# indrajeetadityaroy9/vit-inductive-bias-distillation

Measured on AMD Instinct MI355X. Metric: distillation images/sec (BASD loss fwd+bwd+grad all-reduce), DeiT-S<-ResNet-50 @ bs256/GPU, higher is better.
Workload: dtype f32; 1 GPU; cfg2 DeiT-S<-ResNet-50 224x224; per_gpu_batch=256, global_batch=256, input_dtype=float32, layout=strided (CLS-sliced / channel-major views), backward=True, grad_allreduce_bytes=88202672, grad_allreduce=none at world size 1 (bucket packed, nothing to exchange), rank_readback=auto, readback_deferred_steps=1756, selector=basd_selector_chain mode 0, parallelism=dp1

## Files before the change

### include/basd_hip.h

```cpp
#ifndef BASD_HIP_H
#define BASD_HIP_H

#include <stdint.h>

#ifdef __cplusplus
extern "C" {
#endif

#ifndef __HIP_PLATFORM_AMD__
typedef struct ihipStream_t* hipStream_t;
#endif

#define BASD_OK 0
#define BASD_EINVAL (-1)
#define BASD_EUNSUPPORTED (-2)
#define BASD_DTYPE_F32 0
#define BASD_DTYPE_BF16 1
#define BASD_DTYPE_U8 2


int basd_gemm_nt(const void* a, int a_dtype, long a_sb, long a_sn, long a_sd, int a_rows_per_batch,
                 long a_batch_stride, const float* b, long ldb, long b_batch_stride, int M, int N, int K, int batch,
                 float* c, long ldc, long c_batch_stride, float scale, const float* bias, float beta,
                 float* colsum_part, float* col_mean, hipStream_t stream);
// ... 153 lines not shown
                              const float* omega_t, float* mu, float* tc, hipStream_t stream);
long basd_teacher_center_stream_scratch_floats(int G, int B, int n, int D);
int basd_teacher_center_stream(const void* const* tok_ptrs, int dtype, const float* mix, int L, int G, long sb, long sn,
                               long sd, int B, int n, int D, const int* g0, const int* g1, const float* glam,
                               const float* omega_t, float* mu, float* tc, float* scratch, hipStream_t stream);

int basd_gram_f64(const float* p, long p_batch_stride, int n, int D, int batch, double* g, long g_batch_stride,
                  hipStream_t stream);

int basd_gram_f64_split(const float* p, long p_batch_stride, int n, int D, int batch, int splits, double* slabs,
                        double* g, hipStream_t stream);

int basd_chol_f64(const double* g, long g_batch_stride, int n, int batch, double* l, long l_batch_stride,
                  hipStream_t stream);

int basd_stack_product(const double* la, const double* lb, long l_batch_stride, int n, int batch, int lb_period,
                       float* w, long w_batch_stride, hipStream_t stream);

int basd_procrustes_finalize(const float* w, long w_batch_stride, const float* sigma, int n, int n_s, int batch,
                             int t_period ,
                             const double* gb, long g_batch_stride, const float* omega, const int* tap0,
                             const int* tap1, const float* lam, const float* tr_s_part, int tr_slabs, float* tr_s,
                             float* tr_t, float* nuc, float* loss, float* k_prime, hipStream_t stream);

int basd_student_project_multi(const void* const* x_ptrs, int dtype, long sb, long sn, int E, int B, int n_s, int n_t,
                               int D, int ptrs_16B_aligned, const float* omega, long omega_e_stride, const int* tap0,
                               const int* tap1, const float* lam, const int* range0, const int* range1, float* mu,
                               float* tr_s, float* a_prime, hipStream_t stream);
int basd_student_grad_multi(const void* const* x_ptrs, int dtype, long sb, long sn, int E, int B, int n_s, int n_t,
                            int D, const float* omega, long omega_e_stride, const float* mu, const float* h,
// ... 32 lines not shown
int basd_procrustes_forward_fused(const BasdProcrustesArgs* args, hipStream_t stream);
int basd_procrustes_tuning(int transposed_cores);

int basd_stack_product_t(const double* la, const double* lb, long l_batch_stride, int n, int batch, int lb_period,
                         float* w, long w_batch_stride, hipStream_t stream);
int basd_kprime_from_transposed(const float* w, long w_batch_stride, const float* sigma, int n, int batch,
                                const double* lb, long l_batch_stride, int lb_period, float* z, long z_batch_stride,
                                float* k_prime, hipStream_t stream);
int basd_procrustes_finish_transposed(const float* w, long w_batch_stride, const float* sigma, int n, int n_s,
                                      int batch, int t_period ,
                                      const double* gb, long g_batch_stride, const float* omega, const int* tap0,
                                      const int* tap1, const float* lam, const float* tr_s_part, int tr_slabs,
                                      float* tr_s, float* tr_t, float* nuc, float* loss, const double* lb,
                                      long l_batch_stride, int lb_period, float* k_prime, hipStream_t stream);
int basd_procrustes_finish_tuning(int fused);
int basd_ustack_stash(const float* wc, long wc_batch_stride, int n, int batch, float* w_stack, long w_stack_stride,
                      hipStream_t stream);
int basd_ustack_from_transposed(const float* x, long x_batch_stride, const float* sigma, int n, int batch,
                                float* w_stack, long w_stack_stride, float* scratch, long scratch_batch_stride,
                                float* sigma_u, int max_sweeps, int* jflags, hipStream_t stream);

int basd_scale_unless_one(float* x, long count, const float* num, const float* den, hipStream_t stream);

int basd_cross_entropy(const void* logits, int dtype, long ld, int B, int C, const long* labels, const float* probs,
                       long pld, float label_smoothing, long ignore_index, float* row_loss, float* dlogits,
                       hipStream_t stream);


int basd_event_create(void** out);
int basd_event_destroy(void* event);
// ... 156 lines not shown
```

### vit-inductive-bias-distillation_amd/basd_amd/_lib.py

```python
from __future__ import annotations

import ctypes as C
import os
import threading

_HERE = os.path.dirname(os.path.abspath(__file__))
LIB_PATH = os.path.join(_HERE, "libbasd_hip.so")

vp, i32, i64, f32, f64 = C.c_void_p, C.c_int, C.c_long, C.c_float, C.c_double

SIGNATURES = {
    "basd_gemm_nt": [vp, i32, i64, i64, i64, i32, i64, vp, i64, i64, i32, i32, i32, i32, vp, i64, i64, f32, vp, f32,
                     vp, vp, vp],
    "basd_gemm_tn_splits": [i32],
    "basd_gemm_tn": [vp, vp, i32, i64, i64, i64, i64, i64, i64, i64, i64, i32, i32, i32, i32, i32, vp, vp, i32, vp,
                     vp, i64, i64, f32, vp],
    "basd_colmean_parts": [i32],
    "basd_colmean": [vp, i32, i64, i64, i64, i32, i64, i32, i32, i32, i32, vp, vp, vp],
    "basd_colmean_multi": [vp, i32, i64, i64, i64, i32, i32, i32, i32, i32, vp, vp, i32, vp],
    "basd_syrk_splits": [i32, i32, i32],
    "basd_syrk_multi": [vp, i32, i64, i64, i64, i32, i32, i32, i32, vp, vp, i32, vp, vp, i64, i32, vp, i32, i32, vp],
    "basd_jacobi_workspace_ints": [i32, i32],
    "basd_jacobi_max_rows": [],
    "basd_jacobi_twopass_workspace_bytes": [i32, i32, i32],
# ... 42 lines not shown
                                 vp, vp],
    "basd_student_project_multi": [vp, i32, i64, i64, i32, i32, i32, i32, i32, i32, vp, i64, vp, vp, vp, vp, vp, vp,
                                   vp, vp, vp],
    "basd_student_grad_multi": [vp, i32, i64, i64, i32, i32, i32, i32, i32, vp, i64, vp, vp, vp, vp, vp, vp, f32, vp,
                                vp, vp, vp],
    "basd_student_grad_fused": [vp, i32, i64, i64, i32, i32, i32, i32, i32, i32, vp, i64, vp, vp, vp, vp, vp, vp, vp,
                                f32, vp, vp],
    "basd_procrustes_forward_fused": [vp, vp],
    "basd_procrustes_tuning": [i32],
    "basd_jacobi_plain4_fits": [i32],
    "basd_stack_product_t": [vp, vp, i64, i32, i32, i32, vp, i64, vp],
    "basd_kprime_from_transposed": [vp, i64, vp, i32, i32, vp, i64, i32, vp, i64, vp, vp],
    "basd_procrustes_finish_transposed": [vp, i64, vp, i32, i32, i32, i32, vp, i64, vp, vp, vp, vp, vp, i32, vp, vp, vp,
                                          vp, vp, i64, i32, vp, vp],
    "basd_procrustes_finish_tuning": [i32],
    "basd_ustack_stash": [vp, i64, i32, i32, vp, i64, vp],
    "basd_ustack_from_transposed": [vp, i64, vp, i32, i32, vp, i64, vp, i64, vp, i32, vp, vp],
    "basd_resample_tokens": [vp, i32, i64, i64, i64, i32, i32, i32, i32, vp, vp, vp, vp, vp],
    "basd_resample_tokens_adjoint": [vp, i32, i32, i32, i32, vp, vp, vp, vp, vp, vp, vp],
    "basd_teacher_factor": [vp, i64, vp, i32, i32, i32, vp, vp, i64, vp, vp, vp, vp, vp, vp, vp, vp, vp],
    "basd_teacher_factor_tiled": [vp, i64, vp, i32, i32, i32, vp, vp, i64, vp, vp, vp, vp, vp, vp, vp, vp, vp, vp],
    "basd_mix_grad_tokens": [vp, vp, i32, i32, i64, i64, i64, i32, i32, i32, i32, vp, vp, vp, vp, vp],
    "basd_mix_grad_tokens_scratch_floats": [i32, i32, i32, i32],
    "basd_mix_grad_tokens_onepass": [vp, vp, i32, i32, i64, i64, i64, i32, i32, i32, i32, vp, vp, vp, vp, vp, vp],
    "basd_token_weight_bwd": [vp, vp, i32, i32, i32, i32, vp, vp, vp, vp, vp, vp, i32, i32, i64, i64, i64, i64, i32,
                              i32, i32, vp, vp, vp],
    "basd_build_angle_stack": [vp, i32, vp, i32, vp, vp],
    "basd_grassmann_distance_bwd": [vp, vp, i32, vp, vp, i32, vp, vp, i32, vp, vp],
    "basd_eigvec_k2": [vp, vp, i32, i32, i32, vp, vp],
    "basd_selector_chain": [vp],
# ... 114 lines not shown
```

### vit-inductive-bias-distillation_amd/csrc/fused.hip

```cpp
#include "basd_common.h"
#include "../../include/basd_hip.h"

namespace basd {

__global__ void __launch_bounds__(256) uwso_combine_kernel(const float* __restrict__ ce, const float* __restrict__ loss_b,
                                                           int E, int B, float* __restrict__ out) {
    constexpr int CH = 32;
    __shared__ double red[CH][4];
    const int tid = threadIdx.x;
    double geo_sum = 0.;
    for (int e0 = 0; e0 < E; e0 += CH) {
        const int ne = E - e0 < CH ? E - e0 : CH;
        for (int e = 0; e < ne; ++e) {
            double acc = 0.;
            for (int b = tid; b < B; b += 256) acc += (double)loss_b[(long)(e0 + e) * B + b];
            for (int m = 32; m > 0; m >>= 1) acc += __shfl_xor(acc, m, 64);
            if ((tid & 63) == 0) red[e][tid >> 6] = acc;
        }
        __syncthreads();
        if (tid == 0)
            for (int e = 0; e < ne; ++e) {
                const float layer = (float)(((red[e][0] + red[e][1]) + (red[e][2] + red[e][3])) / (double)B);
                out[4 + E + e0 + e] = layer;
                geo_sum += (double)layer;
// ... 1 lines not shown
        __syncthreads();
    }
    if (tid == 0) {
        const float c = ce[0], geo = (float)(geo_sum / (double)E);
        const float eps = 1.1920929e-7f;
        const float i0 = 1.f / fmaxf(c, eps), i1 = 1.f / fmaxf(geo, eps);
        const float w0 = i0 / (i0 + i1), w1 = i1 / (i0 + i1);
        out[0] = w0;
        out[1] = w1;
        out[2] = w0 * c + w1 * geo;
        out[3] = geo;
        for (int e = 0; e < E; ++e) out[4 + e] = w1 / (float)E;
    }
}

__global__ void __launch_bounds__(256) scale_unless_one_kernel(float* __restrict__ x, long count4, long count,
                                                               const float* __restrict__ num,
                                                               const float* __restrict__ den) {
    const float f = den ? num[0] / den[0] : num[0];
    if (f == 1.f) return;
    const long i = (long)blockIdx.x * 256 + threadIdx.x;
    if (i < count4) {
        float4 v = ((float4*)x)[i];
        v.x *= f; v.y *= f; v.z *= f; v.w *= f;
        ((float4*)x)[i] = v;
    }
    if (blockIdx.x == 0 && threadIdx.x < (int)(count - 4 * count4)) x[4 * count4 + threadIdx.x] *= f;
}

}

extern "C" {

int basd_scale_unless_one(float* x, long count, const float* num, const float* den, hipStream_t stream) {
    BASD_CHECK_ARG(x && num && count > 0 && ((uintptr_t)x & 15) == 0);
    const long count4 = count / 4;
    basd::scale_unless_one_kernel<<<(unsigned)((count4 + 255) / 256 + (count4 == 0)), 256, 0, stream>>>(x, count4, count, num, den);
    BASD_RETURN_LAST();
}

static int procrustes_tail(const BasdProcrustesArgs* a, const float* grad_layers, int E, int B, int n_s, int n, int d_s,
                           int EB, long nn, long om_stride, hipStream_t st) {
    int rc;
#define BASD_TRY(call)            \
    do {                          \
        rc = (call);              \
        if (rc != BASD_OK) return rc; \
    } while (0)
    if (a->uw_ce) {
        BASD_CHECK_ARG(a->uw_out != nullptr);
        basd::uwso_combine_kernel<<<1, 256, 0, st>>>(a->uw_ce, a->loss_b, E, B, a->uw_out);
        grad_layers = a->uw_out + 4;
// ... 65 lines not shown
    rc = basd_student_project_multi(a->student_ptrs, (int)a->s_dtype, a->s_sb, a->s_sn, E, B, n_s, n, d_s,
                                    (int)a->s_aligned, a->omega, om_stride, a->tap0, a->tap1, a->lam, a->range0,
                                    a->range1, a->mu_s, a->tr_part, a->a_prime, st);
    if (rc == BASD_EUNSUPPORTED) {
        slabs = (d_s + 63) / 64;
        for (int e = 0; e < E; ++e)
            BASD_TRY(basd_student_project(a->student_host_ptrs[e], (int)a->s_dtype, a->s_sb, a->s_sn, B, n_s, n, d_s,
                                          a->omega + e * om_stride, a->tap0, a->tap1, a->lam, a->range0, a->range1,
                                          a->mu_s + (long)e * B * d_s, a->tr_part + (long)e * B * slabs,
                                          a->a_prime + (long)e * B * n * d_s, st));
    } else if (rc != BASD_OK) {
        return rc;
    }
    const long nn = (long)n * n;
    const int EB = E * B, GB = G * B;
    BASD_TRY(basd_gram_f64(a->a_prime, (long)n * d_s, n, d_s, EB, a->g_all, nn, st));
    if (a->g_slabs && a->g_splits > 1)
        BASD_TRY(basd_gram_f64_split(a->tc, (long)n * d_t, n, d_t, GB, (int)a->g_splits, a->g_slabs,
                                     a->g_all + (long)EB * nn, st));
    else
        BASD_TRY(basd_gram_f64(a->tc, (long)n * d_t, n, d_t, GB, a->g_all + (long)EB * nn, nn, st));
    BASD_TRY(basd_chol_f64(a->g_all, nn, n, EB + GB, a->l_all, nn, st));
    if ((a->raw == nullptr || a->w_stack != nullptr) && EB <= 65535 && basd_jacobi_plain4_fits(n) &&
        (g_transposed_cores == 2 || (g_transposed_cores == 1 && EB >= 128))) {
        BASD_TRY(basd_stack_product_t(a->l_all, a->l_all + (long)EB * nn, nn, n, EB, GB, a->W, 2 * nn, st));
        if (a->raw != nullptr) BASD_TRY(basd_ustack_stash(a->W, 2 * nn, n, EB, a->w_stack, 2 * nn, st));
        BASD_TRY(basd_jacobi_onesided(a->W, 2 * nn, n, n, n, EB, nullptr, a->sigma, n, (int)a->max_sweeps, 0.f,
                                      a->jflags, a->sweeps, st));
        rc = BASD_EUNSUPPORTED;
        if (a->k_prime && g_finish_fused)
            rc = basd_procrustes_finish_transposed(a->W, 2 * nn, a->sigma, n, n_s, EB, GB, a->g_all + (long)EB * nn, nn,
                                                   a->omega, a->tap0, a->tap1, a->lam, a->tr_part, slabs, a->tr_s,
                                                   a->tr_t, a->nuc, a->loss_b, a->l_all + (long)EB * nn, nn, GB,
                                                   a->k_prime, st);
        if (rc == BASD_EUNSUPPORTED) {
            BASD_TRY(basd_procrustes_finalize(a->W, 2 * nn, a->sigma, n, n_s, EB, GB, a->g_all + (long)EB * nn, nn,
                                              a->omega, a->tap0, a->tap1, a->lam, a->tr_part, slabs, a->tr_s, a->tr_t,
// ... 48 lines not shown
```

### vit-inductive-bias-distillation_amd/csrc/jacobi.hip

```cpp
#include "basd_common.h"

namespace basd {

constexpr float kNull2 = 2.2737368e-13f;

struct Rot {
    float c, s, t;
    float h;
    bool apply;
    bool strong;
};

__device__ __forceinline__ Rot make_rotation(float alpha, float beta, float gamma, float tol) {
    Rot r{1.f, 0.f, 0.f, 0.f, false, false};
    const float cosv = gamma * __builtin_amdgcn_rsqf(alpha) * __builtin_amdgcn_rsqf(beta);
    if (!(fabsf(cosv) > tol)) return r;
    r.strong = cosv * cosv > tol;
    const float zeta = (beta - alpha) * __builtin_amdgcn_rcpf(2.f * gamma);
    const float az = fabsf(zeta);
    float t = az > 1e8f ? 0.5f * __builtin_amdgcn_rcpf(az)
                        : __builtin_amdgcn_rcpf(az + __builtin_amdgcn_sqrtf(fmaf(zeta, zeta, 1.f)));
    t = copysignf(t, zeta);
    r.t = t;
    r.c = __builtin_amdgcn_rsqf(fmaf(t, t, 1.f));
// ... 767 lines not shown
            (void)hipFuncSetAttribute((const void*)jacobi_lds_kernel<20, 20, 8>,
                                      hipFuncAttributeMaxDynamicSharedMemorySize, BASD_JACOBI_LDS_LIMIT);
            jacobi_lds_kernel<20, 20, 8><<<batch, threads, lds8p, stream>>>(W, batch_stride, rows_dot, rows_tot, n, n_arr,
                                                                            max_sweeps, tol, colnorm, colnorm_stride,
                                                                            sweeps_out);
            BASD_RETURN_LAST();
        }
    }

    if (g_jacobi_ordering == 1 && !stacked && !n_arr && n_even >= 8 && rows_tot == rows_dot &&
        (lanes == 0 || lanes == 4) && (g_jacobi_lanes == 4 || (batch >= 128 && n_even >= 40) || n_even >= 96)) {
        static const int o_epl[] = {8, 16, 24, 36, 50};
        int e4 = 0;
        for (int e : o_epl)
            if (4 * e >= rows_tot) { e4 = e; break; }
        const int G = n_even / 2;
        const size_t lds_oe = (size_t)(G + 1) * (plain4_ld(e4) + 2) * sizeof(float);
        const int threads = ((G * 4 + 63) / 64) * 64;
        if (e4 && threads <= 512 && lds_oe <= BASD_JACOBI_LDS_LIMIT) {
#define LAUNCH_OE(E)                                                                                                  \
    do {                                                                                                              \
        if (lds_oe > 48 * 1024)                                                                                       \
            (void)hipFuncSetAttribute((const void*)jacobi_oe_kernel<E>, hipFuncAttributeMaxDynamicSharedMemorySize,   \
                                      BASD_JACOBI_LDS_LIMIT);                                                         \
        jacobi_oe_kernel<E><<<batch, threads, lds_oe, stream>>>(W, batch_stride, rows_tot, n, max_sweeps, tol, colnorm, \
                                                                colnorm_stride, sweeps_out);                          \
    } while (0)
            switch (e4) {
                case 8: LAUNCH_OE(8); break;
                case 16: LAUNCH_OE(16); break;
                case 24: LAUNCH_OE(24); break;
                case 36: LAUNCH_OE(36); break;
                default: LAUNCH_OE(50); break;
            }
#undef LAUNCH_OE
            BASD_RETURN_LAST();
        }
    }

    if (!stacked && !n_arr && n_even >= 8 && (lanes == 4 || (lanes == 0 && batch >= 128 && n_even >= 40))) {
        static const int p_epl[] = {8, 16, 24, 36, 50};
        int e4 = 0;
        for (int e : p_epl)
            if (4 * e >= rows_tot) { e4 = e; break; }
// ... 233 lines not shown
```

### vit-inductive-bias-distillation_amd/csrc/procrustes.hip

```cpp
#include "basd_common.h"
#include "../../include/basd_hip.h"

namespace basd {

typedef double f64x4 __attribute__((ext_vector_type(4)));

template <typename T>
__global__ void __launch_bounds__(256) token_weights_kernel(const void* const* __restrict__ attn_ptrs,
                                                            const float* __restrict__ mix, int L, long sb, long sh,
                                                            long sq, long sk, int H, int A, int has_cls, int n_a,
                                                            int n_t, int n_s, const int* __restrict__ atap0,
                                                            const int* __restrict__ atap1,
                                                            const float* __restrict__ alam,
                                                            const int* __restrict__ tap0,
                                                            const int* __restrict__ tap1,
                                                            const float* __restrict__ lam, float* __restrict__ omega,
                                                            float* __restrict__ omega_t, float* __restrict__ raw_out) {
    extern __shared__ float sm[];
    float* raw = sm;
    float* w = sm + n_a;
    __shared__ float red[32];
    const int b = blockIdx.x, tid = threadIdx.x;
    for (int j = tid; j < n_a; j += blockDim.x) {
        float acc = 0.f;
// ... 6 lines not shown
            }
            acc /= (float)H;
        } else {
            for (int h = 0; h < H; ++h)
                for (int q = 0; q < A; ++q) {
                    float m = 0.f;
                    for (int l = 0; l < L; ++l)
                        m += mix[l] * ldg_f32((const BASD_GLOBAL_AS T*)attn_ptrs[l] + (b * sb + h * sh + q * sq + (long)j * sk));
                    acc += m;
                }
            acc /= (float)(H * A);
        }
        raw[j] = acc;
        if (raw_out) raw_out[(long)b * n_a + j] = acc;
    }
    __syncthreads();
    float part = 0.f;
    for (int n = tid; n < n_s; n += blockDim.x) {
        float v;
        if (atap0) {
            const float l1 = alam[n];
            v = (1.f - l1) * raw[atap0[n]] + l1 * raw[atap1[n]];
        } else {
            v = raw[n];
        }
        w[n] = v;
        part += v;
    }
    const float total = block_sum(part, red);
    for (int n = tid; n < n_s; n += blockDim.x) {
        const float v = w[n] / total;
        w[n] = v;
        omega[(long)b * n_s + n] = v;
    }
    __syncthreads();
    for (int j = tid; j < n_t; j += blockDim.x) {
        float acc = 0.f;
        if (tap0) {
            for (int n = 0; n < n_s; ++n) {
                const float l1 = lam[n];
                if (tap0[n] == j) acc += (1.f - l1) * w[n];
                if (tap1[n] == j) acc += l1 * w[n];
            }
        } else {
            acc = w[j];
        }
        omega_t[(long)b * n_t + j] = acc;
    }
}

template <typename T>
__global__ void __launch_bounds__(256) student_project_kernel(const T* __restrict__ X, long sb, long sn, int n_s,
                                                              int n_t, int D, const float* __restrict__ omega,
                                                              const int* __restrict__ tap0,
                                                              const int* __restrict__ tap1,
                                                              const float* __restrict__ lam,
                                                              const int* __restrict__ range0,
                                                              const int* __restrict__ range1,
                                                              float* __restrict__ mu_out, float* __restrict__ tr_part,
                                                              float* __restrict__ Ap) {
    extern __shared__ float sm[];
    float* w = sm;
    __shared__ float red[4][64];
// ... 376 lines not shown
                                                                   int D, float* __restrict__ mu_out,
                                                                   float* __restrict__ Tc) {
    const int d = blockIdx.x * 256 + threadIdx.x, chunk = blockIdx.y;
    const long gb = blockIdx.z, GB = gridDim.z;
    if (d >= D) return;
    float mu = 0.f;
    for (int c = 0; c < chunks; ++c) mu += chunk_sum[((long)c * GB + gb) * D + d];
    if (chunk == 0) mu_out[gb * D + d] = mu;
    const int j_lo = chunk * TCS_ROWS, j_hi = j_lo + TCS_ROWS < n ? j_lo + TCS_ROWS : n;
    float* out = Tc + gb * n * D + d;
    for (int j = j_lo; j < j_hi; ++j) out[(long)j * D] -= mu;
}

constexpr int G64_BK = 32, G64_LD = 36, G64_TPW = 8;

__global__ void __launch_bounds__(1024) gram_f64_kernel(const float* __restrict__ P, long p_batch_stride, int n, int D,
                                                        double* __restrict__ G, long g_batch_stride,
                                                        long g_split_stride) {
    extern __shared__ __attribute__((aligned(16))) float tile[];
    const int b = blockIdx.x, tid = threadIdx.x, lane = tid & 63, wave = tid >> 6, nw = blockDim.x >> 6;
    G += (long)blockIdx.y * g_split_stride;
    const int nt = (n + 15) / 16, ntiles = nt * (nt + 1) / 2;
    const float* Pb = P + (long)b * p_batch_stride;
    f64x4 acc[G64_TPW];
#pragma unroll
    for (int t = 0; t < G64_TPW; ++t) acc[t] = f64x4{0., 0., 0., 0.};
    int ti[G64_TPW], tj[G64_TPW];
#pragma unroll
    for (int t = 0; t < G64_TPW; ++t) {
        const int lin = wave + (t + (int)blockIdx.z * G64_TPW) * nw;
        int r = 0;
        if (lin < ntiles) {
            r = (int)((sqrtf(8.f * lin + 1.f) - 1.f) * 0.5f);
            while ((r + 1) * (r + 2) / 2 <= lin) ++r;
            while (r * (r + 1) / 2 > lin) --r;
            ti[t] = r;
            tj[t] = lin - r * (r + 1) / 2;
        } else {
            ti[t] = -1;
            tj[t] = -1;
        }
    }
    const int rows_pad = nt * 16;
    const int i16 = lane & 15, kq = lane >> 4;
    for (int k0 = blockIdx.y * G64_BK; k0 < D; k0 += G64_BK * gridDim.y) {
        __syncthreads();
        for (int idx = tid; idx < rows_pad * (G64_BK / 4); idx += blockDim.x) {
            const int r = idx / (G64_BK / 4), c4 = (idx - r * (G64_BK / 4)) * 4, k = k0 + c4;
            float4 v = make_float4(0.f, 0.f, 0.f, 0.f);
            if (r < n) {
                const float* p = Pb + (long)r * D + k;
                if (k + 3 < D) {
                    v = *(const float4*)p;
                } else {
                    if (k < D) v.x = p[0];
                    if (k + 1 < D) v.y = p[1];
                    if (k + 2 < D) v.z = p[2];
                }
            }
            *(float4*)(tile + r * G64_LD + c4) = v;
        }
        __syncthreads();
#pragma unroll
        for (int g = 0; g < G64_BK / 16; ++g) {
#pragma unroll
            for (int t = 0; t < G64_TPW; ++t) {
                if (ti[t] < 0) continue;
                const float4 a = *(const float4*)(tile + (ti[t] * 16 + i16) * G64_LD + g * 16 + 4 * kq);
                const float4 bb = *(const float4*)(tile + (tj[t] * 16 + i16) * G64_LD + g * 16 + 4 * kq);
                acc[t] = __builtin_amdgcn_mfma_f64_16x16x4f64((double)a.x, (double)bb.x, acc[t], 0, 0, 0);
                acc[t] = __builtin_amdgcn_mfma_f64_16x16x4f64((double)a.y, (double)bb.y, acc[t], 0, 0, 0);
                acc[t] = __builtin_amdgcn_mfma_f64_16x16x4f64((double)a.z, (double)bb.z, acc[t], 0, 0, 0);
                acc[t] = __builtin_amdgcn_mfma_f64_16x16x4f64((double)a.w, (double)bb.w, acc[t], 0, 0, 0);
            }
        }
    }
    double* Gb = G + (long)b * g_batch_stride;
#pragma unroll
    for (int t = 0; t < G64_TPW; ++t) {
        if (ti[t] < 0) continue;
        const int col = tj[t] * 16 + (lane & 15);
#pragma unroll
        for (int r = 0; r < 4; ++r) {
            const int row = ti[t] * 16 + (lane >> 4) + 4 * r;
            if (row < n && col < n) {
                Gb[(long)row * n + col] = acc[t][r];
                Gb[(long)col * n + row] = acc[t][r];
            }
        }
    }
}

__global__ void __launch_bounds__(256) gram_f64_reduce_kernel(const double* __restrict__ slabs, long split_stride,
                                                              int splits, long count, double* __restrict__ G) {
    const long i = (long)blockIdx.x * 256 + threadIdx.x;
    if (i >= count) return;
    double acc = 0.;
    for (int s2 = 0; s2 < splits; ++s2) acc += slabs[(long)s2 * split_stride + i];
    G[i] = acc;
}

static bool gram_f64_shape(int n, int* waves, int* chunks, size_t* lds) {
    const int nt = (n + 15) / 16, ntiles = nt * (nt + 1) / 2;
    int w = (ntiles + G64_TPW - 1) / G64_TPW;
    if (w < 4) w = ntiles < 4 ? ntiles : 4;
// ... 1 lines not shown
    if (w > 16) {
        c = (ntiles + 16 * G64_TPW - 1) / (16 * G64_TPW);
        w = 16;
    }
    *waves = w;
    *chunks = c;
    *lds = sizeof(float) * (size_t)nt * 16 * G64_LD;
    if (*lds > 156 * 1024) return false;
    if (*lds > 48 * 1024)
        (void)hipFuncSetAttribute((const void*)gram_f64_kernel, hipFuncAttributeMaxDynamicSharedMemorySize, 156 * 1024);
    return true;
}

__device__ __forceinline__ int pk(int i, int j, int n) { return j * n - (j * (j - 1)) / 2 + (i - j); }

__global__ void __launch_bounds__(1024) chol_f64_kernel(const double* __restrict__ G, long g_batch_stride, int n,
                                                        double* __restrict__ Lout, long l_batch_stride) {
    extern __shared__ __attribute__((aligned(16))) double a[];
    double* col = a + (size_t)n * (n + 1) / 2;
    __shared__ double sh_piv;
    __shared__ double red[32];
    const int m = blockIdx.x, tid = threadIdx.x, nthr = blockDim.x, lane = tid & 63, wave = tid >> 6, nw = nthr >> 6;
    const double* Gm = G + (long)m * g_batch_stride;
    double dmax = 0.;
    for (int j = wave; j < n; j += nw)
        for (int i = j + lane; i < n; i += 64) {
            const double v = Gm[(long)i * n + j];
            a[pk(i, j, n)] = v;
            if (i == j) dmax = fmax(dmax, v);
        }
    for (int s = 32; s > 0; s >>= 1) dmax = fmax(dmax, __shfl_xor(dmax, s, 64));
    if (lane == 0) red[wave] = dmax;
    __syncthreads();
    dmax = 0.;
    for (int i = 0; i < nw; ++i) dmax = fmax(dmax, red[i]);
    const double thr = dmax * (double)n * 1e-15;
    for (int j = 0; j < n; ++j) {
        if (tid == 0) {
            const double d = a[pk(j, j, n)];
            sh_piv = d > thr ? sqrt(d) : 0.;
        }
        __syncthreads();
        const double piv = sh_piv;
        const double inv = piv > 0. ? 1. / piv : 0.;
        for (int i = j + tid; i < n; i += nthr) {
// ... 713 lines not shown
    for (int d = threadIdx.x; d < D; d += 128) {
        float acc = 0.f;
        for (int s = s0; s < s1; ++s) {
            const float l1 = lam[s];
            const float coef = (tap0[s] == j ? 1.f - l1 : 0.f) + (tap1[s] == j ? l1 : 0.f);
            acc = fmaf(coef, dY[((long)b * n_out + s) * D + d], acc);
        }
        dX[((long)b * n_in + j) * D + d] = acc;
    }
}

}

using namespace basd;

extern "C" {

int basd_token_weights(const void* const* attn_ptrs, int dtype, const float* mix, int L, long sb, long sh, long sq,
                       long sk, int B, int H, int A, int has_cls, int n_a, int n_t, int n_s, const int* atap0,
                       const int* atap1, const float* alam, const int* tap0, const int* tap1, const float* lam,
                       float* omega, float* omega_t, float* raw_out, hipStream_t stream) {
    BASD_CHECK_ARG(attn_ptrs && mix && omega && omega_t && L > 0 && B > 0 && H > 0 && n_a > 0 && n_t > 0 && n_s > 0);
    BASD_CHECK_ARG(A == n_a + (has_cls ? 1 : 0));
    BASD_CHECK_ARG((n_a == n_s) == (atap0 == nullptr));
    BASD_CHECK_ARG((n_t == n_s) == (tap0 == nullptr));
    const size_t lds = sizeof(float) * (size_t)(n_a + n_s);
    if (dtype == BASD_DTYPE_F32)
        token_weights_kernel<float><<<B, 256, lds, stream>>>(attn_ptrs, mix, L, sb, sh, sq, sk, H, A, has_cls, n_a, n_t, n_s, atap0, atap1, alam, tap0, tap1, lam, omega, omega_t, raw_out);
    else if (dtype == BASD_DTYPE_BF16)
        token_weights_kernel<__hip_bfloat16><<<B, 256, lds, stream>>>(attn_ptrs, mix, L, sb, sh, sq, sk, H, A, has_cls, n_a, n_t, n_s, atap0, atap1, alam, tap0, tap1, lam, omega, omega_t, raw_out);
    else
        return BASD_EINVAL;
    BASD_RETURN_LAST();
}

int basd_student_project(const void* x, int dtype, long sb, long sn, int B, int n_s, int n_t, int D,
                         const float* omega, const int* tap0, const int* tap1, const float* lam, const int* range0,
                         const int* range1, float* mu, float* tr_s, float* a_prime, hipStream_t stream) {
    BASD_CHECK_ARG(x && omega && mu && tr_s && a_prime && B > 0 && n_s > 0 && n_t > 0 && D > 0);
    BASD_CHECK_ARG((n_t == n_s) == (tap0 == nullptr));
// ... 192 lines not shown
    gram_f64_reduce_kernel<<<(unsigned)((count + 255) / 256), 256, 0, stream>>>(slabs, count, splits, count, g);
    BASD_RETURN_LAST();
}

int basd_chol_f64(const double* g, long g_batch_stride, int n, int batch, double* l, long l_batch_stride,
                  hipStream_t stream) {
    BASD_CHECK_ARG(g && l && n > 0 && batch > 0);
    const size_t lds = sizeof(double) * ((size_t)n * (n + 1) / 2 + n);
    if (lds > 158 * 1024) {
        if (n > 64 * CB_MAXR) return BASD_EUNSUPPORTED;
        const size_t lds_b = sizeof(double) * ((size_t)n * CB_NB + (size_t)CB_NB * (CB_KC + 1));
        (void)hipFuncSetAttribute((const void*)chol_f64_blocked_kernel, hipFuncAttributeMaxDynamicSharedMemorySize, 156 * 1024);
        chol_f64_blocked_kernel<<<batch, 1024, lds_b, stream>>>(g, g_batch_stride, n, l, l_batch_stride);
        BASD_RETURN_LAST();
    }
    (void)hipFuncSetAttribute((const void*)chol_f64_kernel, hipFuncAttributeMaxDynamicSharedMemorySize, 158 * 1024);
    const int threads = n >= 128 ? 1024 : n >= 64 ? 512 : 256;
    chol_f64_kernel<<<batch, threads, lds, stream>>>(g, g_batch_stride, n, l, l_batch_stride);
    BASD_RETURN_LAST();
}

int basd_stack_product(const double* la, const double* lb, long l_batch_stride, int n, int batch, int lb_period,
                       float* w, long w_batch_stride, hipStream_t stream) {
    BASD_CHECK_ARG(la && lb && w && n > 0 && batch > 0 && lb_period > 0);
    const size_t lds = sizeof(double) * 2 * (size_t)n * n;
    if (lds <= 78 * 1024) {
        (void)hipFuncSetAttribute((const void*)stack_product_kernel, hipFuncAttributeMaxDynamicSharedMemorySize, 78 * 1024);
        stack_product_kernel<<<batch, 256, lds, stream>>>(la, lb, l_batch_stride, n, w, w_batch_stride, lb_period);
    } else {
        BASD_CHECK_ARG(batch <= 65535);
        const int nt = (n + 31) / 32;
        stack_product_global_kernel<<<dim3(nt, nt, batch), 256, 0, stream>>>(la, lb, l_batch_stride, n, w, w_batch_stride, lb_period);
    }
// ... 177 lines not shown
```

Before: 170,400 images/s.

## Fuse paired Gram launches, fold split reduction into Cholesky, stage token weights

Student and teacher f64 Gram computations now run as one combined launch, with a small-TPW variant when there are few tiles. The split-slab reduction moves into the Cholesky kernel, which sums the slabs while loading. Token weights gain a staged LDS kernel with unrolled loads, the scale kernel becomes grid-stride with a capped grid, and the Jacobi odd-even path gets an extra e4=14 specialization. The aim is fewer launches and better memory-level parallelism. The cost is more code paths and redundant summation in the fold path.

```diff
diff --git a/include/basd_hip.h b/include/basd_hip.h
--- a/include/basd_hip.h
+++ b/include/basd_hip.h
@@ -191,6 +191,12 @@
 int basd_chol_f64(const double* g, long g_batch_stride, int n, int batch, double* l, long l_batch_stride,
                   hipStream_t stream);
 
+int basd_gram_f64_pair(const float* p0, long p0_batch_stride, int d0, int batch0, double* g0, long g0_batch_stride,
+                       const float* p1, long p1_batch_stride, int d1, int batch1, int splits1, double* out1,
+                       long out1_batch_stride, int n, hipStream_t stream);
+int basd_chol_f64_fold(double* g, long g_batch_stride, int n, int batch, int fold_from, const double* slabs, int splits,
+                       double* l, long l_batch_stride, hipStream_t stream);
+
 int basd_stack_product(const double* la, const double* lb, long l_batch_stride, int n, int batch, int lb_period,
                        float* w, long w_batch_stride, hipStream_t stream);
 
@@ -253,6 +259,7 @@
                                       float* tr_s, float* tr_t, float* nuc, float* loss, const double* lb,
                                       long l_batch_stride, int lb_period, float* k_prime, hipStream_t stream);
 int basd_procrustes_finish_tuning(int fused);
+int basd_procrustes_launch_tuning(int mask);
 int basd_ustack_stash(const float* wc, long wc_batch_stride, int n, int batch, float* w_stack, long w_stack_stride,
                       hipStream_t stream);
 int basd_ustack_from_transposed(const float* x, long x_batch_stride, const float* sigma, int n, int batch,
diff --git a/vit-inductive-bias-distillation_amd/basd_amd/_lib.py b/vit-inductive-bias-distillation_amd/basd_amd/_lib.py
--- a/vit-inductive-bias-distillation_amd/basd_amd/_lib.py
+++ b/vit-inductive-bias-distillation_amd/basd_amd/_lib.py
@@ -80,6 +80,9 @@
     "basd_procrustes_finish_transposed": [vp, i64, vp, i32, i32, i32, i32, vp, i64, vp, vp, vp, vp, vp, i32, vp, vp, vp,
                                           vp, vp, i64, i32, vp, vp],
     "basd_procrustes_finish_tuning": [i32],
+    "basd_procrustes_launch_tuning": [i32],
+    "basd_gram_f64_pair": [vp, i64, i32, i32, vp, i64, vp, i64, i32, i32, i32, vp, i64, i32, vp],
+    "basd_chol_f64_fold": [vp, i64, i32, i32, i32, vp, i32, vp, i64, vp],
     "basd_ustack_stash": [vp, i64, i32, i32, vp, i64, vp],
     "basd_ustack_from_transposed": [vp, i64, vp, i32, i32, vp, i64, vp, i64, vp, i32, vp, vp],
     "basd_resample_tokens": [vp, i32, i64, i64, i64, i32, i32, i32, i32, vp, vp, vp, vp, vp],
diff --git a/vit-inductive-bias-distillation_amd/csrc/fused.hip b/vit-inductive-bias-distillation_amd/csrc/fused.hip
--- a/vit-inductive-bias-distillation_amd/csrc/fused.hip
+++ b/vit-inductive-bias-distillation_amd/csrc/fused.hip
@@ -39,13 +39,13 @@
     }
 }
 
+constexpr int SCALE_MAX_BLOCKS = 2048;
 __global__ void __launch_bounds__(256) scale_unless_one_kernel(float* __restrict__ x, long count4, long count,
                                                                const float* __restrict__ num,
                                                                const float* __restrict__ den) {
     const float f = den ? num[0] / den[0] : num[0];
     if (f == 1.f) return;
-    const long i = (long)blockIdx.x * 256 + threadIdx.x;
-    if (i < count4) {
+    for (long i = (long)blockIdx.x * 256 + threadIdx.x; i < count4; i += (long)gridDim.x * 256) {
         float4 v = ((float4*)x)[i];
         v.x *= f; v.y *= f; v.z *= f; v.w *= f;
         ((float4*)x)[i] = v;
@@ -60,7 +60,9 @@
 int basd_scale_unless_one(float* x, long count, const float* num, const float* den, hipStream_t stream) {
     BASD_CHECK_ARG(x && num && count > 0 && ((uintptr_t)x & 15) == 0);
     const long count4 = count / 4;
-    basd::scale_unless_one_kernel<<<(unsigned)((count4 + 255) / 256 + (count4 == 0)), 256, 0, stream>>>(x, count4, count, num, den);
+    long blocks = (count4 + 255) / 256 + (count4 == 0);
+    if (blocks > basd::SCALE_MAX_BLOCKS) blocks = basd::SCALE_MAX_BLOCKS;
+    basd::scale_unless_one_kernel<<<(unsigned)blocks, 256, 0, stream>>>(x, count4, count, num, den);
     BASD_RETURN_LAST();
 }
 
@@ -156,13 +158,27 @@
     }
     const long nn = (long)n * n;
     const int EB = E * B, GB = G * B;
-    BASD_TRY(basd_gram_f64(a->a_prime, (long)n * d_s, n, d_s, EB, a->g_all, nn, st));
-    if (a->g_slabs && a->g_splits > 1)
-        BASD_TRY(basd_gram_f64_split(a->tc, (long)n * d_t, n, d_t, GB, (int)a->g_splits, a->g_slabs,
-                                     a->g_all + (long)EB * nn, st));
-    else
-        BASD_TRY(basd_gram_f64(a->tc, (long)n * d_t, n, d_t, GB, a->g_all + (long)EB * nn, nn, st));
-    BASD_TRY(basd_chol_f64(a->g_all, nn, n, EB + GB, a->l_all, nn, st));
+    const int launch_mask = basd_procrustes_launch_tuning(-1);
+    const bool split = a->g_slabs && a->g_splits > 1;
+    rc = BASD_EUNSUPPORTED;
+    if (launch_mask & 2)
+        rc = basd_gram_f64_pair(a->a_prime, (long)n * d_s, d_s, EB, a->g_all, nn, a->tc, (long)n * d_t, d_t, GB,
+                                split ? (int)a->g_splits : 1, split ? a->g_slabs : a->g_all + (long)EB * nn, nn, n, st);
+    if (rc == BASD_OK && split) {
+        BASD_TRY(basd_chol_f64_fold(a->g_all, nn, n, EB + GB, EB, a->g_slabs, (int)a->g_splits, a->l_all, nn, st));
+    } else {
+        if (rc == BASD_EUNSUPPORTED) {
+            BASD_TRY(basd_gram_f64(a->a_prime, (long)n * d_s, n, d_s, EB, a->g_all, nn, st));
+            if (split)
+                BASD_TRY(basd_gram_f64_split(a->tc, (long)n * d_t, n, d_t, GB, (int)a->g_splits, a->g_slabs,
+                                             a->g_all + (long)EB * nn, st));
+            else
+                BASD_TRY(basd_gram_f64(a->tc, (long)n * d_t, n, d_t, GB, a->g_all + (long)EB * nn, nn, st));
+        } else if (rc != BASD_OK) {
+            return rc;
+        }
+        BASD_TRY(basd_chol_f64(a->g_all, nn, n, EB + GB, a->l_all, nn, st));
+    }
     if ((a->raw == nullptr || a->w_stack != nullptr) && EB <= 65535 && basd_jacobi_plain4_fits(n) &&
         (g_transposed_cores == 2 || (g_transposed_cores == 1 && EB >= 128))) {
         BASD_TRY(basd_stack_product_t(a->l_all, a->l_all + (long)EB * nn, nn, n, EB, GB, a->W, 2 * nn, st));
diff --git a/vit-inductive-bias-distillation_amd/csrc/jacobi.hip b/vit-inductive-bias-distillation_amd/csrc/jacobi.hip
--- a/vit-inductive-bias-distillation_amd/csrc/jacobi.hip
+++ b/vit-inductive-bias-distillation_amd/csrc/jacobi.hip
@@ -805,6 +805,7 @@
         int e4 = 0;
         for (int e : o_epl)
             if (4 * e >= rows_tot) { e4 = e; break; }
+        if (e4 == 16 && rows_tot > 48 && rows_tot <= 56) e4 = 14;
         const int G = n_even / 2;
         const size_t lds_oe = (size_t)(G + 1) * (plain4_ld(e4) + 2) * sizeof(float);
         const int threads = ((G * 4 + 63) / 64) * 64;
@@ -819,6 +820,7 @@
     } while (0)
             switch (e4) {
                 case 8: LAUNCH_OE(8); break;
+                case 14: LAUNCH_OE(14); break;
                 case 16: LAUNCH_OE(16); break;
                 case 24: LAUNCH_OE(24); break;
                 case 36: LAUNCH_OE(36); break;
diff --git a/vit-inductive-bias-distillation_amd/csrc/procrustes.hip b/vit-inductive-bias-distillation_amd/csrc/procrustes.hip
--- a/vit-inductive-bias-distillation_amd/csrc/procrustes.hip
+++ b/vit-inductive-bias-distillation_amd/csrc/procrustes.hip
@@ -4,6 +4,47 @@
 namespace basd {
 
 typedef double f64x4 __attribute__((ext_vector_type(4)));
+
+__device__ __forceinline__ void token_weights_finish(const float* raw, float* w, float* red, int b, int tid, int n_a,
+                                                     int n_t, int n_s, const int* __restrict__ atap0,
+                                                     const int* __restrict__ atap1, const float* __restrict__ alam,
+                                                     const int* __restrict__ tap0, const int* __restrict__ tap1,
+                                                     const float* __restrict__ lam, float* __restrict__ omega,
+                                                     float* __restrict__ omega_t) {
+    __syncthreads();
+    float part = 0.f;
+    for (int n = tid; n < n_s; n += blockDim.x) {
+        float v;
+        if (atap0) {
+            const float l1 = alam[n];
+            v = (1.f - l1) * raw[atap0[n]] + l1 * raw[atap1[n]];
+        } else {
+            v = raw[n];
+        }
+        w[n] = v;
+        part += v;
+    }
+    const float total = block_sum(part, red);
+    for (int n = tid; n < n_s; n += blockDim.x) {
+        const float v = w[n] / total;
+        w[n] = v;
+        omega[(long)b * n_s + n] = v;
+    }
+    __syncthreads();
+    for (int j = tid; j < n_t; j += blockDim.x) {
+        float acc = 0.f;
+        if (tap0) {
+            for (int n = 0; n < n_s; ++n) {
+                const float l1 = lam[n];
+                if (tap0[n] == j) acc += (1.f - l1) * w[n];
+                if (tap1[n] == j) acc += l1 * w[n];
+            }
+        } else {
+            acc = w[j];
+        }
+        omega_t[(long)b * n_t + j] = acc;
+    }
+}
 
 template <typename T>
 __global__ void __launch_bounds__(256) token_weights_kernel(const void* const* __restrict__ attn_ptrs,
@@ -44,39 +85,67 @@
         raw[j] = acc;
         if (raw_out) raw_out[(long)b * n_a + j] = acc;
     }
-    __syncthreads();
-    float part = 0.f;
-    for (int n = tid; n < n_s; n += blockDim.x) {
-        float v;
-        if (atap0) {
-            const float l1 = alam[n];
-            v = (1.f - l1) * raw[atap0[n]] + l1 * raw[atap1[n]];
-        } else {
-            v = raw[n];
-        }
-        w[n] = v;
-        part += v;
-    }
-    const float total = block_sum(part, red);
-    for (int n = tid; n < n_s; n += blockDim.x) {
-        const float v = w[n] / total;
-        w[n] = v;
-        omega[(long)b * n_s + n] = v;
-    }
-    __syncthreads();
-    for (int j = tid; j < n_t; j += blockDim.x) {
-        float acc = 0.f;
-        if (tap0) {
-            for (int n = 0; n < n_s; ++n) {
-                const float l1 = lam[n];
-                if (tap0[n] == j) acc += (1.f - l1) * w[n];
-                if (tap1[n] == j) acc += l1 * w[n];
-            }
-        } else {
-            acc = w[j];
-        }
-        omega_t[(long)b * n_t + j] = acc;
-    }
+    token_weights_finish(raw, w, red, b, tid, n_a, n_t, n_s, atap0, atap1, alam, tap0, tap1, lam, omega, omega_t);
+}
+
+constexpr int TW_UNROLL = 10, TW_STAGE = 256 * TW_UNROLL;
+template <typename T>
+__global__ void __launch_bounds__(256) token_weights_staged_kernel(
+    const void* const* __restrict__ attn_ptrs, const float* __restrict__ mix, int L, long sb, long sh, long sq, long sk,
+    int H, int A, int has_cls, int n_a, int n_t, int n_s, const int* __restrict__ atap0, const int* __restrict__ atap1,
+    const float* __restrict__ alam, const int* __restrict__ tap0, const int* __restrict__ tap1,
+    const float* __restrict__ lam, float* __restrict__ omega, float* __restrict__ omega_t, float* __restrict__ raw_out) {
+    extern __shared__ float sm[];
+    float* raw = sm;
+    float* w = sm + n_a;
+    float* stage = w + n_s;
+    __shared__ float red[32];
+    const int b = blockIdx.x, tid = threadIdx.x;
+    const int rows = has_cls ? H : H * A, col0 = has_cls ? 1 : 0;
+    const int rows_pass = TW_STAGE / n_a;
+    float acc[TW_UNROLL];
+#pragma unroll
+    for (int u = 0; u < TW_UNROLL; ++u) acc[u] = 0.f;
+    for (int r0 = 0; r0 < rows; r0 += rows_pass) {
+        const int nr = rows - r0 < rows_pass ? rows - r0 : rows_pass, count = nr * n_a;
+        float m[TW_UNROLL];
+        long off[TW_UNROLL];
+#pragma unroll
+        for (int u = 0; u < TW_UNROLL; ++u) {
+            const int e = tid + 256 * u, r = e / n_a, j = e - r * n_a, row = r0 + r;
+            const int h = has_cls ? row : row / A, q = has_cls ? 0 : row - h * A;
+            off[u] = b * sb + h * sh + q * sq + (long)(col0 + j) * sk;
+            m[u] = 0.f;
+        }
+        for (int l = 0; l < L; ++l) {
+            const BASD_GLOBAL_AS T* base = (const BASD_GLOBAL_AS T*)attn_ptrs[l];
+            const float ml = mix[l];
+#pragma unroll
+            for (int u = 0; u < TW_UNROLL; ++u)
+                if (tid + 256 * u < count) m[u] += ml * ldg_f32(base + off[u]);
+        }
+        __syncthreads();
+#pragma unroll
+        for (int u = 0; u < TW_UNROLL; ++u)
+            if (tid + 256 * u < count) stage[tid + 256 * u] = m[u];
+        __syncthreads();
+#pragma unroll
+        for (int u = 0; u < TW_UNROLL; ++u) {
+            const int j = tid + 256 * u;
+            if (j < n_a)
+                for (int r = 0; r < nr; ++r) acc[u] += stage[r * n_a + j];
+        }
+    }
+#pragma unroll
+    for (int u = 0; u < TW_UNROLL; ++u) {
+        const int j = tid + 256 * u;
+        if (j < n_a) {
+            const float v = acc[u] / (float)rows;
+            raw[j] = v;
+            if (raw_out) raw_out[(long)b * n_a + j] = v;
+        }
+    }
+    token_weights_finish(raw, w, red, b, tid, n_a, n_t, n_s, atap0, atap1, alam, tap0, tap1, lam, omega, omega_t);
 }
 
 template <typename T>
@@ -483,21 +552,22 @@
 
 constexpr int G64_BK = 32, G64_LD = 36, G64_TPW = 8;
 
-__global__ void __launch_bounds__(1024) gram_f64_kernel(const float* __restrict__ P, long p_batch_stride, int n, int D,
-                                                        double* __restrict__ G, long g_batch_stride,
-                                                        long g_split_stride) {
+template <int TPW>
+__device__ __forceinline__ void gram_f64_block(const float* __restrict__ P, long p_batch_stride, int n, int D,
+                                               double* __restrict__ G, long g_batch_stride, long g_split_stride, int b,
+                                               int split, int splits, int zchunk) {
     extern __shared__ __attribute__((aligned(16))) float tile[];
-    const int b = blockIdx.x, tid = threadIdx.x, lane = tid & 63, wave = tid >> 6, nw = blockDim.x >> 6;
-    G += (long)blockIdx.y * g_split_stride;
+    const int tid = threadIdx.x, lane = tid & 63, wave = tid >> 6, nw = blockDim.x >> 6;
+    G += (long)split * g_split_stride;
     const int nt = (n + 15) / 16, ntiles = nt * (nt + 1) / 2;
     const float* Pb = P + (long)b * p_batch_stride;
-    f64x4 acc[G64_TPW];
-#pragma unroll
-    for (int t = 0; t < G64_TPW; ++t) acc[t] = f64x4{0., 0., 0., 0.};
-    int ti[G64_TPW], tj[G64_TPW];
-#pragma unroll
-    for (int t = 0; t < G64_TPW; ++t) {
-        const int lin = wave + (t + (int)blockIdx.z * G64_TPW) * nw;
+    f64x4 acc[TPW];
+#pragma unroll
+    for (int t = 0; t < TPW; ++t) acc[t] = f64x4{0., 0., 0., 0.};
+    int ti[TPW], tj[TPW];
+#pragma unroll
+    for (int t = 0; t < TPW; ++t) {
+        const int lin = wave + (t + zchunk * TPW) * nw;
         int r = 0;
         if (lin < ntiles) {
             r = (int)((sqrtf(8.f * lin + 1.f) - 1.f) * 0.5f);
@@ -512,7 +582,7 @@
     }
     const int rows_pad = nt * 16;
     const int i16 = lane & 15, kq = lane >> 4;
-    for (int k0 = blockIdx.y * G64_BK; k0 < D; k0 += G64_BK * gridDim.y) {
+    for (int k0 = split * G64_BK; k0 < D; k0 += G64_BK * splits) {
         __syncthreads();
         for (int idx = tid; idx < rows_pad * (G64_BK / 4); idx += blockDim.x) {
             const int r = idx / (G64_BK / 4), c4 = (idx - r * (G64_BK / 4)) * 4, k = k0 + c4;
@@ -533,7 +603,7 @@
 #pragma unroll
         for (int g = 0; g < G64_BK / 16; ++g) {
 #pragma unroll
-            for (int t = 0; t < G64_TPW; ++t) {
+            for (int t = 0; t < TPW; ++t) {
                 if (ti[t] < 0) continue;
                 const float4 a = *(const float4*)(tile + (ti[t] * 16 + i16) * G64_LD + g * 16 + 4 * kq);
                 const float4 bb = *(const float4*)(tile + (tj[t] * 16 + i16) * G64_LD + g * 16 + 4 * kq);
@@ -546,7 +616,7 @@
     }
     double* Gb = G + (long)b * g_batch_stride;
 #pragma unroll
-    for (int t = 0; t < G64_TPW; ++t) {
+    for (int t = 0; t < TPW; ++t) {
         if (ti[t] < 0) continue;
         const int col = tj[t] * 16 + (lane & 15);
 #pragma unroll
@@ -558,6 +628,31 @@
             }
         }
     }
+}
+
+__global__ void __launch_bounds__(1024) gram_f64_kernel(const float* __restrict__ P, long p_batch_stride, int n, int D,
+                                                        double* __restrict__ G, long g_batch_stride,
+                                                        long g_split_stride) {
+    gram_f64_block<G64_TPW>(P, p_batch_stride, n, D, G, g_batch_stride, g_split_stride, blockIdx.x, blockIdx.y, gridDim.y,
+                            blockIdx.z);
+}
+
+struct GramSeg {
+    const float* P;
+    double* G;
+    long p_batch_stride, g_batch_stride, g_split_stride;
+    int D, batch, splits, blocks;
+};
+template <int TPW>
+__global__ void __launch_bounds__(TPW <= 3 ? 256 : 1024) gram_f64_kernel_pair(GramSeg first, GramSeg second, int n) {
+    const bool lead = (int)blockIdx.x < first.blocks;
+    const int i = lead ? (int)blockIdx.x : (int)blockIdx.x - first.blocks;
+    const int batch = lead ? first.batch : second.batch, split = i / batch, b = i - split * batch;
+    gram_f64_block<TPW>(lead ? first.P : second.P, lead ? first.p_batch_stride : second.p_batch_stride, n,
+                        lead ? first.D : second.D, lead ? first.G : second.G,
+                        lead ? first.g_batch_stride : second.g_batch_stride,
+                        lead ? first.g_split_stride : second.g_split_stride, b, split,
+                        lead ? first.splits : second.splits, 0);
 }
 
 __global__ void __launch_bounds__(256) gram_f64_reduce_kernel(const double* __restrict__ slabs, long split_stride,
@@ -589,21 +684,36 @@
 
 __device__ __forceinline__ int pk(int i, int j, int n) { return j * n - (j * (j - 1)) / 2 + (i - j); }
 
-__global__ void __launch_bounds__(1024) chol_f64_kernel(const double* __restrict__ G, long g_batch_stride, int n,
-                                                        double* __restrict__ Lout, long l_batch_stride) {
+template <bool FOLD>
+__global__ void __launch_bounds__(1024) chol_f64_kernel(double* __restrict__ G, long g_batch_stride, int n,
+                                                        double* __restrict__ Lout, long l_batch_stride, int fold_from,
+                                                        const double* __restrict__ slabs, long split_stride,
+                                                        int splits) {
     extern __shared__ __attribute__((aligned(16))) double a[];
     double* col = a + (size_t)n * (n + 1) / 2;
     __shared__ double sh_piv;
     __shared__ double red[32];
     const int m = blockIdx.x, tid = threadIdx.x, nthr = blockDim.x, lane = tid & 63, wave = tid >> 6, nw = nthr >> 6;
-    const double* Gm = G + (long)m * g_batch_stride;
+    double* Gm = G + (long)m * g_batch_stride;
     double dmax = 0.;
-    for (int j = wave; j < n; j += nw)
-        for (int i = j + lane; i < n; i += 64) {
-            const double v = Gm[(long)i * n + j];
-            a[pk(i, j, n)] = v;
+    if (FOLD && m >= fold_from) {
+        const double* sl = slabs + (long)(m - fold_from) * n * n;
+        for (int idx = tid; idx < n * n; idx += nthr) {
+            const int i = idx / n, j = idx - i * n;
+            double v = 0.;
+            for (int s2 = 0; s2 < splits; ++s2) v += sl[(long)s2 * split_stride + idx];
+            Gm[idx] = v;
+            if (i >= j) a[pk(i, j, n)] = v;
             if (i == j) dmax = fmax(dmax, v);
         }
+    } else {
+        for (int j = wave; j < n; j += nw)
+            for (int i = j + lane; i < n; i += 64) {
+                const double v = Gm[(long)i * n + j];
+                a[pk(i, j, n)] = v;
+                if (i == j) dmax = fmax(dmax, v);
+            }
+    }
     for (int s = 32; s > 0; s >>= 1) dmax = fmax(dmax, __shfl_xor(dmax, s, 64));
     if (lane == 0) red[wave] = dmax;
     __syncthreads();
@@ -1347,7 +1457,15 @@
 
 using namespace basd;
 
+static int g_launch_mask = 3;
+
 extern "C" {
+
+int basd_procrustes_launch_tuning(int mask) {
+    const int prev = g_launch_mask;
+    if (mask >= 0) g_launch_mask = mask & 3;
+    return prev;
+}
 
 int basd_token_weights(const void* const* attn_ptrs, int dtype, const float* mix, int L, long sb, long sh, long sq,
                        long sk, int B, int H, int A, int has_cls, int n_a, int n_t, int n_s, const int* atap0,
@@ -1357,6 +1475,16 @@
     BASD_CHECK_ARG(A == n_a + (has_cls ? 1 : 0));
     BASD_CHECK_ARG((n_a == n_s) == (atap0 == nullptr));
     BASD_CHECK_ARG((n_t == n_s) == (tap0 == nullptr));
+    const size_t lds_st = sizeof(float) * ((size_t)n_a + n_s + TW_STAGE);
+    if ((g_launch_mask & 1) && n_a <= TW_STAGE && lds_st <= 48 * 1024) {
+        if (dtype == BASD_DTYPE_F32)
+            token_weights_staged_kernel<float><<<B, 256, lds_st, stream>>>(attn_ptrs, mix, L, sb, sh, sq, sk, H, A, has_cls, n_a, n_t, n_s, atap0, atap1, alam, tap0, tap1, lam, omega, omega_t, raw_out);
+        else if (dtype == BASD_DTYPE_BF16)
+            token_weights_staged_kernel<__hip_bfloat16><<<B, 256, lds_st, stream>>>(attn_ptrs, mix, L, sb, sh, sq, sk, H, A, has_cls, n_a, n_t, n_s, atap0, atap1, alam, tap0, tap1, lam, omega, omega_t, raw_out);
+        else
+            return BASD_EINVAL;
+        BASD_RETURN_LAST();
+    }
     const size_t lds = sizeof(float) * (size_t)(n_a + n_s);
     if (dtype == BASD_DTYPE_F32)
         token_weights_kernel<float><<<B, 256, lds, stream>>>(attn_ptrs, mix, L, sb, sh, sq, sk, H, A, has_cls, n_a, n_t, n_s, atap0, atap1, alam, tap0, tap1, lam, omega, omega_t, raw_out);
@@ -1579,9 +1707,51 @@
         chol_f64_blocked_kernel<<<batch, 1024, lds_b, stream>>>(g, g_batch_stride, n, l, l_batch_stride);
         BASD_RETURN_LAST();
     }
-    (void)hipFuncSetAttribute((const void*)chol_f64_kernel, hipFuncAttributeMaxDynamicSharedMemorySize, 158 * 1024);
+    (void)hipFuncSetAttribute((const void*)chol_f64_kernel<false>, hipFuncAttributeMaxDynamicSharedMemorySize, 158 * 1024);
     const int threads = n >= 128 ? 1024 : n >= 64 ? 512 : 256;
-    chol_f64_kernel<<<batch, threads, lds, stream>>>(g, g_batch_stride, n, l, l_batch_stride);
+    chol_f64_kernel<false><<<batch, threads, lds, stream>>>((double*)g, g_batch_stride, n, l, l_batch_stride, batch, nullptr, 0, 0);
+    BASD_RETURN_LAST();
+}
+
+int basd_gram_f64_pair(const float* p0, long p0_batch_stride, int d0, int batch0, double* g0, long g0_batch_stride,
+                       const float* p1, long p1_batch_stride, int d1, int batch1, int splits1, double* out1,
+                       long out1_batch_stride, int n, hipStream_t stream) {
+    BASD_CHECK_ARG(p0 && g0 && p1 && out1 && n > 0 && d0 > 0 && d1 > 0 && batch0 > 0 && batch1 > 0 && splits1 >= 1 &&
+                   splits1 <= 64);
+    BASD_CHECK_ARG(((uintptr_t)p0 & 15) == 0 && d0 % 4 == 0 && p0_batch_stride % 4 == 0);
+    BASD_CHECK_ARG(((uintptr_t)p1 & 15) == 0 && d1 % 4 == 0 && p1_batch_stride % 4 == 0);
+    BASD_CHECK_ARG(splits1 == 1 || out1_batch_stride == (long)n * n);
+    int waves, chunks;
+    size_t lds;
+    if (!gram_f64_shape(n, &waves, &chunks, &lds) || chunks != 1) return BASD_EUNSUPPORTED;
+    const long blocks = (long)batch0 + (long)batch1 * splits1;
+    if (blocks > 0x7fffffffL) return BASD_EUNSUPPORTED;
+    GramSeg s0{p0, g0, p0_batch_stride, g0_batch_stride, 0, d0, batch0, 1, batch0};
+    GramSeg s1{p1, out1, p1_batch_stride, out1_batch_stride, (long)batch1 * out1_batch_stride, d1, batch1, splits1,
+               batch1 * splits1};
+    const int c0 = (d0 + G64_BK - 1) / G64_BK, c1 = ((d1 + G64_BK - 1) / G64_BK + splits1 - 1) / splits1;
+    const bool swap = c1 > c0;
+    const int nt = (n + 15) / 16, ntiles = nt * (nt + 1) / 2;
+    if ((ntiles + waves - 1) / waves <= 3)
+        gram_f64_kernel_pair<3><<<(unsigned)blocks, 64 * waves, lds, stream>>>(swap ? s1 : s0, swap ? s0 : s1, n);
+    else
+        gram_f64_kernel_pair<G64_TPW><<<(unsigned)blocks, 64 * waves, lds, stream>>>(swap ? s1 : s0, swap ? s0 : s1, n);
+    BASD_RETURN_LAST();
+}
+
+int basd_chol_f64_fold(double* g, long g_batch_stride, int n, int batch, int fold_from, const double* slabs, int splits,
+                       double* l, long l_batch_stride, hipStream_t stream) {
+    BASD_CHECK_ARG(g && l && slabs && n > 0 && batch > 0 && fold_from >= 0 && fold_from < batch && splits >= 1);
+    const long nn = (long)n * n, count = (long)(batch - fold_from) * nn;
+    const size_t lds = sizeof(double) * ((size_t)n * (n + 1) / 2 + n);
+    if (lds > 158 * 1024) {
+        BASD_CHECK_ARG(g_batch_stride == nn);
+        gram_f64_reduce_kernel<<<(unsigned)((count + 255) / 256), 256, 0, stream>>>(slabs, count, splits, count, g + (long)fold_from * nn);
+        return basd_chol_f64(g, g_batch_stride, n, batch, l, l_batch_stride, stream);
+    }
+    (void)hipFuncSetAttribute((const void*)chol_f64_kernel<true>, hipFuncAttributeMaxDynamicSharedMemorySize, 158 * 1024);
+    const int threads = n >= 128 ? 1024 : n >= 64 ? 512 : 256;
+    chol_f64_kernel<true><<<batch, threads, lds, stream>>>(g, g_batch_stride, n, l, l_batch_stride, fold_from, slabs, count, splits);
     BASD_RETURN_LAST();
 }
 
```

New measurement: 159,600 images/s. 6.3% lower.
